# BadgerTechnologies/navigation

Measured on NVIDIA B200. Metric: ms per updateMap+inflation @4k^2 grid; DWA trajectories scored/sec, lower is better.
Workload: dtype u8

## Files before the change

### navigation_b200/csrc/dwa.cu

```cuda
#include <algorithm>
#include <cmath>
#include <cstdlib>
#include <limits>
#include <memory>
#include <vector>

#include "dwa_kernels.cuh"
#include "fleet_costmap.cuh"
#include "tp_kernels.cuh"

using namespace navgpu;

namespace {

struct P2 {
  double x, y;
};

void adjust_plan_resolution(const std::vector<P2>& in, std::vector<P2>& out, double resolution) {
  out.clear();
  if (in.empty()) return;
  double last_x = in[0].x, last_y = in[0].y;
  out.push_back(in[0]);
  const double min_sq_resolution = resolution * resolution * 4;
// ... 88 lines not shown
    NAVGPU_CUDA(cudaEventCreateWithFlags(ev, cudaEventDisableTiming));
  } else {
    NAVGPU_CUDA(cudaEventSynchronize(*ev));
  }
  memcpy(*stage, host_grid, bytes);
  NAVGPU_CUDA(cudaMemcpy2DAsync(dev, pitch, *stage, sx, sx, sy, cudaMemcpyHostToDevice, stream));
  NAVGPU_CUDA(cudaEventRecord(*ev, stream));
  return NAVGPU_OK;
}
}

struct navgpu_dwa {
  int device = 0;
  cudaStream_t stream = nullptr;
  navgpu_dwa_config cfg;
  unsigned sx = 0, sy = 0;
  double res = 0;
  uint8_t* d_cost_own = nullptr;
  const uint8_t* d_cost = nullptr;
  uint8_t* h_cost_stage = nullptr;
  cudaEvent_t ev_cost_stage = nullptr;
  unsigned pitch = 0;
  double ox = 0, oy = 0;
  DwaPlans plans;
  double* d_plan[3] = {nullptr, nullptr, nullptr};
  size_t plan_capacity[3] = {0, 0, 0};
  bool plan_dirty[3] = {false, false, false};
  bool align_aliased = false;
  DwaScales scales = {};
  uint32_t* d_dist[4] = {nullptr, nullptr, nullptr, nullptr};
  float* d_samples = nullptr;
  size_t samples_capacity = 0;
  float* h_samples_stage = nullptr;
  size_t samples_stage_capacity = 0;
  cudaEvent_t ev_samples_stage = nullptr;
  bool samples_on_device = false;
  double* d_block_cost = nullptr;
  long long* d_block_index = nullptr;
  size_t block_capacity = 0;
  unsigned int* d_counters = nullptr;
  double* d_best_cost = nullptr;
  long long* d_best_index = nullptr;
  DwaDeviceResult* h_result = nullptr;
  double* h_points = nullptr;
  double* h_best = nullptr;
  double* d_terms = nullptr;
// ... 80 lines not shown
    auto launch = [&](auto kernel) -> int {
      if (sliced_smem > 48 * 1024)
        NAVGPU_CUDA(cudaFuncSetAttribute(kernel, cudaFuncAttributeMaxDynamicSharedMemorySize, (int)sliced_smem));
      kernel<<<n_ctas, kMapGridThreads, sliced_smem, stream>>>(ma, jobs_per_robot, planes);
      return NAVGPU_OK;
    };
    switch (wpt) {
      case 1: NAVGPU_TRY(launch(k_mapgrid_prepare_sliced<1>)); break;
      case 2: NAVGPU_TRY(launch(k_mapgrid_prepare_sliced<2>)); break;
      case 3: NAVGPU_TRY(launch(k_mapgrid_prepare_sliced<3>)); break;
      default: NAVGPU_TRY(launch(k_mapgrid_prepare_sliced<4>)); break;
    }
  } else {
    const size_t mg_smem = size_t(4) * NW * sizeof(uint32_t);
    if (mg_smem > 200 * 1024) return fail(NAVGPU_ERR_UNSUPPORTED, "local costmap %ux%u too large for the MapGrid kernel", sx, sy);
    if (mg_smem > 48 * 1024)
      NAVGPU_CUDA(cudaFuncSetAttribute(k_mapgrid_prepare, cudaFuncAttributeMaxDynamicSharedMemorySize, (int)mg_smem));
    k_mapgrid_prepare<<<n_ctas, kMapGridThreads, mg_smem, stream>>>(ma, jobs_per_robot);
  }
  NAVGPU_LAUNCHED(1);
  return NAVGPU_OK;
}

int prepare_grids(navgpu_dwa* h, const DwaGeom& g) {
  for (int k = 0; k < 3; ++k) NAVGPU_TRY(upload_plan(h, k));
  MapGridArgs ma;
  ma.g = g;
  ma.allow_unknown = h->cfg.allow_unknown;
  const std::vector<P2>* adjusted = h->plans.adjusted;
  ma.job[0] = MapGridJob{h->d_plan[0], (int)adjusted[0].size(), 0, h->d_dist[0]};
  ma.job[1] = MapGridJob{h->d_plan[0], (int)adjusted[0].size(), 1, h->d_dist[1]};
  ma.job[2] = MapGridJob{h->d_plan[1], (int)adjusted[1].size(), 1, h->d_dist[2]};
  ma.job[3] = MapGridJob{h->d_plan[2], (int)adjusted[2].size(), 0, h->d_dist[3]};
  if (h->plans.align_is_path) {
    ma.job[3].dist = h->d_dist[0];
    ma.job[3].skip = 1;
  }
  ma.fleet = nullptr;
  NAVGPU_TRY(launch_mapgrid(h->sx, h->sy, h->stream, ma, 4, 4));
  h->align_aliased = h->plans.align_is_path;
  return NAVGPU_OK;
}

int critic_args(navgpu_dwa* h, const DwaGeom& g, const double* footprint_xy, int n_footprint, DwaScoreArgs& a) {
  if (n_footprint < 0 || n_footprint > kMaxFootprint) return fail(NAVGPU_ERR_UNSUPPORTED, "footprint with more than %d vertices", kMaxFootprint);
  dwa_config_args(h->cfg, h->scales, footprint_xy, n_footprint, a);
  a.scale_alignment = h->plans.alignment_scale;
  a.g = g;
  for (int k = 0; k < 4; ++k) a.dist[k] = h->d_dist[k];
  if (h->align_aliased) a.dist[3] = h->d_dist[0];
  a.osc_mask = h->osc.mask();
  return NAVGPU_OK;
}

int begin_cycle(navgpu_dwa* h, const double pose[3], const double velv[3], const double* footprint_xy, int n_footprint,
                Cycle& cy, bool prepare = true) {
  NAVGPU_TRY(use_device(h));
  if (!h->d_cost) return fail(NAVGPU_ERR_INVALID, "no costmap set");
  if (h->plans.plan.empty()) return fail(NAVGPU_ERR_INVALID, "no plan set");
  if (n_footprint < 0 || n_footprint > kMaxFootprint) return fail(NAVGPU_ERR_UNSUPPORTED, "footprint with more than %d vertices", kMaxFootprint);
  const float pos[3] = {(float)pose[0], (float)pose[1], (float)pose[2]};
  const float vel[3] = {(float)velv[0], (float)velv[1], (float)velv[2]};
  const float goal[2] = {(float)h->plans.plan.back().x, (float)h->plans.plan.back().y};
// ... 9 lines not shown
    }
    if (!h->samples_on_device || s.v != h->last_samples) {
      const size_t bytes = s.v.size() * sizeof(float);
      if (bytes > h->samples_stage_capacity) {
        if (h->h_samples_stage) cudaFreeHost(h->h_samples_stage);
        h->h_samples_stage = nullptr;
        NAVGPU_CUDA(cudaMallocHost(&h->h_samples_stage, 2 * bytes));
        h->samples_stage_capacity = 2 * bytes;
      }
      if (!h->ev_samples_stage) NAVGPU_CUDA(cudaEventCreateWithFlags(&h->ev_samples_stage, cudaEventDisableTiming));
      else NAVGPU_CUDA(cudaEventSynchronize(h->ev_samples_stage));
      memcpy(h->h_samples_stage, s.v.data(), bytes);
      NAVGPU_CUDA(cudaMemcpyAsync(h->d_samples, h->h_samples_stage, bytes, cudaMemcpyHostToDevice, h->stream));
      NAVGPU_CUDA(cudaEventRecord(h->ev_samples_stage, h->stream));
      h->samples_on_device = true;
    }
  } else {
    h->samples_on_device = false;
  }
  h->last_samples = s.v;
  h->last_nx = s.nx; h->last_ny = s.ny; h->last_nth = s.nth;

  DwaGeom g{h->d_cost, h->sx, h->sy, h->pitch, h->res, h->ox, h->oy, 1.0 / h->res};
  if (prepare) NAVGPU_TRY(prepare_grids(h, g));

  DwaScoreArgs& a = cy.args;
  NAVGPU_TRY(critic_args(h, g, footprint_xy, n_footprint, a));
  a.vxs = h->d_samples;
  a.vys = h->d_samples + s.nx;
  a.vths = h->d_samples + s.nx + s.ny;
  a.nx = s.nx; a.ny = s.ny; a.nth = s.nth;
  a.inline_samples = inline_samples ? 1 : 0;
  if (inline_samples) memcpy(a.samples_inline, s.v.data(), s.v.size() * sizeof(float));
  cy.n_samples = (long long)s.nx * s.ny * s.nth;
  a.begin = 0;
  a.end = cy.n_samples;
  a.stride_rank = 0;
  a.stride_world = 1;
  for (int k = 0; k < kShardMaxWorld; ++k) a.shard_peer[k] = nullptr;
  a.shard_seq = 0;
  for (int k = 0; k < 3; ++k) { a.pos[k] = pos[k]; a.vel[k] = vel[k]; }
  a.all_terms = nullptr;
  a.counters = h->d_counters;
  a.best_cost = h->d_best_cost;
  a.best_index = h->d_best_index;
  a.finish_out = nullptr;
  a.finish_points = nullptr;
  a.finish_capacity = 0;
  h->n_samples_last = cy.n_samples;
  return NAVGPU_OK;
// ... 56 lines not shown
  h->device = device;
  h->cfg = *cfg;
  h->sx = size_x; h->sy = size_y; h->res = resolution;
  NAVGPU_CUDA(cudaSetDevice(device));
  NAVGPU_CUDA(cudaStreamCreateWithFlags(&h->stream, cudaStreamNonBlocking));
  for (int k = 0; k < 4; ++k) NAVGPU_CUDA(cudaMalloc(&h->d_dist[k], size_t(size_x) * size_y * sizeof(uint32_t)));
  NAVGPU_CUDA(cudaMalloc(&h->d_counters, 2 * sizeof(unsigned int)));
  NAVGPU_CUDA(cudaMemset(h->d_counters, 0, 2 * sizeof(unsigned int)));
  NAVGPU_CUDA(cudaMalloc(&h->d_best_cost, sizeof(double)));
  NAVGPU_CUDA(cudaMalloc(&h->d_best_index, sizeof(long long)));
  NAVGPU_CUDA(cudaHostAlloc(&h->h_result, sizeof(DwaDeviceResult), cudaHostAllocMapped));
  NAVGPU_CUDA(cudaHostAlloc(&h->h_points, size_t(kPointsCapacity) * 3 * sizeof(double), cudaHostAllocMapped));
  NAVGPU_CUDA(cudaMallocHost(&h->h_best, 2 * sizeof(double)));
  apply_config(h.get());
  *out = h.release();
  return NAVGPU_OK;
}

int navgpu_dwa_destroy(navgpu_dwa* h) {
  if (!h) return NAVGPU_OK;
  cudaSetDevice(h->device);
  cudaStreamSynchronize(h->stream);
  cudaFree(h->d_cost_own);
  if (h->h_cost_stage) cudaFreeHost(h->h_cost_stage);
  if (h->h_samples_stage) cudaFreeHost(h->h_samples_stage);
  if (h->ev_samples_stage) cudaEventDestroy(h->ev_samples_stage);
  if (h->ev_cost_stage) cudaEventDestroy(h->ev_cost_stage);
  for (int k = 0; k < 3; ++k) cudaFree(h->d_plan[k]);
  for (int k = 0; k < 4; ++k) cudaFree(h->d_dist[k]);
  cudaFree(h->d_samples); cudaFree(h->d_block_cost); cudaFree(h->d_block_index); cudaFree(h->d_counters);
  cudaFree(h->d_best_cost); cudaFree(h->d_best_index);
  cudaFree(h->d_terms); cudaFree(h->d_reported);
  for (int r = 0; r < kShardMaxWorld; ++r)
    if (h->shard_ipc[r] && h->shard_peer[r]) cudaIpcCloseMemHandle(h->shard_peer[r]);
  cudaFree(h->d_shard);
  cudaFree(h->d_traj);
  cudaFreeHost(h->h_result); cudaFreeHost(h->h_points); cudaFreeHost(h->h_best);
  cudaStreamDestroy(h->stream);
  delete h;
  return NAVGPU_OK;
}

int navgpu_dwa_reconfigure(navgpu_dwa* h, const navgpu_dwa_config* cfg) {
  if (!h || !cfg) return fail(NAVGPU_ERR_INVALID, "bad arguments");
  h->cfg = *cfg;
  apply_config(h);
  return NAVGPU_OK;
}

int navgpu_dwa_set_costmap(navgpu_dwa* h, const uint8_t* host_grid, double origin_x, double origin_y) {
  if (!h || !host_grid) return fail(NAVGPU_ERR_INVALID, "bad arguments");
  NAVGPU_TRY(use_device(h));
  const unsigned pitch = grid_pitch(h->sx);
  if (!h->d_cost_own) NAVGPU_CUDA(cudaMalloc(&h->d_cost_own, size_t(pitch) * h->sy));
  NAVGPU_TRY(stage_grid_upload(&h->h_cost_stage, &h->ev_cost_stage, h->d_cost_own, pitch, host_grid, h->sx, h->sy, h->stream));
  h->d_cost = h->d_cost_own;
  h->pitch = pitch;
  h->ox = origin_x;
  h->oy = origin_y;
  return NAVGPU_OK;
}

int navgpu_dwa_set_costmap_device(navgpu_dwa* h, const uint8_t* dev_grid, uint32_t pitch, double origin_x, double origin_y) {
  if (!h || !dev_grid || pitch < h->sx) return fail(NAVGPU_ERR_INVALID, "bad arguments");
  h->d_cost = dev_grid;
  h->pitch = pitch;
  h->ox = origin_x;
  h->oy = origin_y;
  return NAVGPU_OK;
}

int navgpu_dwa_set_plan(navgpu_dwa* h, const double pose[3], const double* plan_xy, int n) {
  if (!h || !pose || !plan_xy || n <= 0) return fail(NAVGPU_ERR_INVALID, "bad plan");
  if (update_plan_and_local_costs(h->plans, h->cfg, h->res, pose, plan_xy, n)) h->plan_dirty[2] = true;
  h->plan_dirty[0] = h->plan_dirty[1] = true;
  return NAVGPU_OK;
}

int navgpu_dwa_reset_oscillation(navgpu_dwa* h) {
  if (!h) return fail(NAVGPU_ERR_INVALID, "null handle");
  h->osc.reset();
  return NAVGPU_OK;
// ... 109 lines not shown
    if (offsets[t + 1] < offsets[t]) return fail(NAVGPU_ERR_INVALID, "trajectory offsets must not decrease");
  const size_t b_points = size_t(n_points) * 3 * sizeof(double), b_vels = size_t(n_traj) * 3 * sizeof(double),
               b_costs = size_t(n_traj) * sizeof(double), b_terms = terms_out ? size_t(n_traj) * 6 * sizeof(double) : 0,
               b_off = size_t(n_traj + 1) * sizeof(int32_t);
  const size_t need = b_points + b_vels + b_costs + b_terms + b_off;
  if (need > h->traj_capacity) {
    if (h->d_traj) cudaFree(h->d_traj);
    h->d_traj = nullptr;
    NAVGPU_CUDA(cudaMalloc(&h->d_traj, 2 * need));
    h->traj_capacity = 2 * need;
  }
  double* d_points = reinterpret_cast<double*>(h->d_traj);
  double* d_vels = reinterpret_cast<double*>(h->d_traj + b_points);
  double* d_costs = reinterpret_cast<double*>(h->d_traj + b_points + b_vels);
  double* d_terms = terms_out ? reinterpret_cast<double*>(h->d_traj + b_points + b_vels + b_costs) : nullptr;
  int* d_off = reinterpret_cast<int*>(h->d_traj + b_points + b_vels + b_costs + b_terms);
  if (b_points) NAVGPU_CUDA(cudaMemcpyAsync(d_points, points_xyth, b_points, cudaMemcpyHostToDevice, h->stream));
  NAVGPU_CUDA(cudaMemcpyAsync(d_vels, vels, b_vels, cudaMemcpyHostToDevice, h->stream));
  NAVGPU_CUDA(cudaMemcpyAsync(d_off, offsets, b_off, cudaMemcpyHostToDevice, h->stream));
  DwaScoreArgs a;
  memset(&a, 0, sizeof(a));
  const DwaGeom g{h->d_cost, h->sx, h->sy, h->pitch, h->res, h->ox, h->oy, 1.0 / h->res};
  NAVGPU_TRY(critic_args(h, g, footprint_xy, n_footprint, a));
  const int blocks = (n_traj + kDwaWarpsPerBlock - 1) / kDwaWarpsPerBlock;
  k_dwa_score_points<<<blocks, kDwaWarpsPerBlock * 32, 0, h->stream>>>(a, d_off, d_points, d_vels, n_traj, d_costs, d_terms);
  NAVGPU_LAUNCHED(1);
  NAVGPU_CUDA(cudaGetLastError());
  NAVGPU_CUDA(cudaMemcpyAsync(costs_out, d_costs, b_costs, cudaMemcpyDeviceToHost, h->stream));
  if (terms_out) NAVGPU_CUDA(cudaMemcpyAsync(terms_out, d_terms, b_terms, cudaMemcpyDeviceToHost, h->stream));
  NAVGPU_CUDA(cudaStreamSynchronize(h->stream));
  return NAVGPU_OK;
}

int navgpu_dwa_update_oscillation(navgpu_dwa* h, const double pose[3], double cost, double xv, double yv, double thetav) {
  if (!h || !pose) return fail(NAVGPU_ERR_INVALID, "bad arguments");
  const float pos[3] = {(float)pose[0], (float)pose[1], (float)pose[2]};
  h->osc.update(pos, cost, xv, yv, thetav, h->cfg.min_trans_vel, h->cfg.oscillation_reset_dist, h->cfg.oscillation_reset_angle);
  return NAVGPU_OK;
}

int navgpu_dwa_get_samples(navgpu_dwa* h, int32_t counts_out[3], float* samples_out, int capacity) {
  if (!h || !counts_out || capacity < 0 || (capacity > 0 && !samples_out)) return fail(NAVGPU_ERR_INVALID, "bad arguments");
  counts_out[0] = h->last_nx; counts_out[1] = h->last_ny; counts_out[2] = h->last_nth;
  const size_t n = std::min<size_t>(h->last_samples.size(), (size_t)capacity);
  if (n) memcpy(samples_out, h->last_samples.data(), n * sizeof(float));
  return h->last_samples.size() > (size_t)capacity ? fail(NAVGPU_ERR_CAPACITY, "samples_out too small") : NAVGPU_OK;
// ... 259 lines not shown
  double* d_block_cost = nullptr;
  long long* d_block_index = nullptr;
  size_t blocks_capacity = 0;
  unsigned* d_generated = nullptr;
  DwaDeviceResult* d_results = nullptr;
  DwaDeviceResult* h_results = nullptr;
  bool plans_dirty = true;
  std::vector<FleetRobot> h_robots;
  std::vector<size_t> plan_off;
  bool started = false;
  FleetTp* tp = nullptr;
  std::vector<uint8_t> active;
  FleetDwaState* h_state = nullptr;
  FleetDwaState* d_state = nullptr;
  bool state_on_device = false;
  float* d_slot_samples = nullptr;
  uint8_t* d_flags = nullptr;
  char* h_records_stage = nullptr;
  cudaEvent_t ev_records_stage = nullptr;
  bool records_dirty = true;
  std::vector<FleetRobot> h_check;
  char* d_check = nullptr;
  size_t check_capacity = 0;
};

static void init_planner_scalars(navgpu_fleet* f, int n_robots, const navgpu_dwa_config* cfg, uint32_t size_x,
                                 uint32_t size_y, double resolution, const double* footprint_xy, int n_footprint,
                                 int device) {
  f->device = device;
  f->n = n_robots;
  f->sx = size_x; f->sy = size_y;
  f->res = resolution;
  f->cfg = *cfg;
  f->footprint.assign(footprint_xy, footprint_xy + 2 * n_footprint);
  f->scales = dwa_scales(*cfg, resolution);
}

static int alloc_planner_side(navgpu_fleet* f) {
  const int n_robots = f->n;
  NAVGPU_CUDA(cudaSetDevice(f->device));
  NAVGPU_CUDA(cudaMalloc(&f->d_robots, sizeof(FleetRobot) * n_robots));
  NAVGPU_CUDA(cudaMalloc(&f->d_dist, size_t(n_robots) * 4 * f->sx * f->sy * sizeof(uint32_t)));
  NAVGPU_CUDA(cudaMalloc(&f->d_generated, sizeof(unsigned) * n_robots));
  NAVGPU_CUDA(cudaMemset(f->d_generated, 0, sizeof(unsigned) * n_robots));
  NAVGPU_CUDA(cudaMalloc(&f->d_results, sizeof(DwaDeviceResult) * n_robots));
  NAVGPU_CUDA(cudaMallocHost(&f->h_results, sizeof(DwaDeviceResult) * n_robots));
// ... 47 lines not shown
  NAVGPU_CUDA(cudaStreamSynchronize(stream));
  return NAVGPU_OK;
}

template <class SetJobs>
static int fleet_upload_grids(navgpu_fleet* f, SetJobs set_jobs) {
  if (!f->grids_dirty) return NAVGPU_OK;
  for (int r = 0; r < f->n; ++r) {
    MapGridRobot& G = f->h_robots[r].grids;
    G.g = DwaGeom{f->d_master + size_t(r) * f->stride * f->pitch, f->sx, f->sy, f->pitch, f->res, f->origins[2 * r],
                  f->origins[2 * r + 1], 1.0 / f->res};
    set_jobs(r, G.job);
  }
  NAVGPU_CUDA(cudaMemcpyAsync(f->d_robots, f->h_robots.data(), sizeof(FleetRobot) * f->n, cudaMemcpyHostToDevice, f->stream));
  NAVGPU_CUDA(cudaStreamSynchronize(f->stream));
  f->grids_dirty = false;
  return NAVGPU_OK;
}

static void fleet_dwa_base_args(const navgpu_fleet* f, DwaScoreArgs& base) {
  memset(&base, 0, sizeof(base));
  base.g = DwaGeom{nullptr, f->sx, f->sy, f->pitch, f->res, 0.0, 0.0, 1.0 / f->res};
  dwa_config_args(f->cfg, f->scales, f->footprint.data(), (int)(f->footprint.size() / 2), base);
}

static int fleet_launch_mapgrid(navgpu_fleet* f, int allow_unknown, int jobs_per_robot) {
  MapGridArgs ma;
  memset(&ma, 0, sizeof(ma));
  ma.g = DwaGeom{nullptr, f->sx, f->sy, f->pitch, f->res, 0.0, 0.0, 1.0 / f->res};
  ma.allow_unknown = allow_unknown;
  ma.fleet = f->d_robots;
  return launch_mapgrid(f->sx, f->sy, f->stream, ma, jobs_per_robot * f->n, jobs_per_robot);
}

static int fleet_state_to_host(navgpu_fleet* f) {
  if (!f->state_on_device) return NAVGPU_OK;
  NAVGPU_CUDA(cudaSetDevice(f->device));
  NAVGPU_CUDA(cudaMemcpyAsync(f->h_state, f->d_state, sizeof(FleetDwaState) * f->n, cudaMemcpyDeviceToHost, f->stream));
  NAVGPU_CUDA(cudaStreamSynchronize(f->stream));
  f->state_on_device = false;
  if (f->sensing) {
    for (int r = 0; r < f->n; ++r) {
      f->origins[2 * r] = f->h_state[r].origin[0];
      f->origins[2 * r + 1] = f->h_state[r].origin[1];
    }
    fleet_costmap_set_origins(f->sensing, f->origins.data());
// ... 85 lines not shown

int navgpu_fleet_create_sensing(navgpu_fleet** out, int n_robots, const navgpu_dwa_config* cfg, uint32_t size_x,
                                uint32_t size_y, double resolution, const navgpu_fleet_costmap_config* cm,
                                const double* footprint_xy, int n_footprint, int device) {
  return create_sensing(out, n_robots, cfg, size_x, size_y, resolution, cm, nullptr, footprint_xy, n_footprint, device);
}

int navgpu_fleet_create_sensing_voxel(navgpu_fleet** out, int n_robots, const navgpu_dwa_config* cfg, uint32_t size_x,
                                      uint32_t size_y, double resolution, const navgpu_fleet_costmap_config* cm,
                                      const navgpu_fleet_voxel_config* voxel, const double* footprint_xy,
                                      int n_footprint, int device) {
  if (!voxel) return fail(NAVGPU_ERR_INVALID, "null voxel config");
  return create_sensing(out, n_robots, cfg, size_x, size_y, resolution, cm, voxel, footprint_xy, n_footprint, device);
}


int navgpu_fleet_destroy(navgpu_fleet* f) {
  if (!f) return NAVGPU_OK;
  cudaSetDevice(f->device);
  if (f->stream) cudaStreamSynchronize(f->stream);
  cudaFree(f->d_stage); cudaFree(f->d_raw); cudaFree(f->d_robots); cudaFree(f->d_plans); cudaFree(f->d_samples); cudaFree(f->d_dist);
  cudaFree(f->d_block_cost); cudaFree(f->d_block_index); cudaFree(f->d_generated); cudaFree(f->d_results);
  cudaFree(f->d_check);
  cudaFreeHost(f->h_results);
  cudaFree(f->d_state); cudaFree(f->d_slot_samples); cudaFree(f->d_flags);
  if (f->h_state) cudaFreeHost(f->h_state);
  if (f->h_records_stage) cudaFreeHost(f->h_records_stage);
  if (f->ev_records_stage) cudaEventDestroy(f->ev_records_stage);
  fleet_tp_free(f->tp);
  navgpu_costmap_destroy(f->costmap);
  fleet_costmap_destroy(f->sensing);
  delete f;
  return NAVGPU_OK;
}

int navgpu_fleet_set_maps(navgpu_fleet* f, const uint8_t* raw_maps, const double* origins_xy) {
  if (!f || !raw_maps || !origins_xy) return fail(NAVGPU_ERR_INVALID, "bad arguments");
  if (f->sensing) return fail(NAVGPU_ERR_INVALID, "a sensing fleet builds its maps from scans (navgpu_fleet_set_scans)");
  NAVGPU_CUDA(cudaSetDevice(f->device));
  f->origins.assign(origins_xy, origins_xy + size_t(2) * f->n);
  f->grids_dirty = true;
  f->records_dirty = true;
  const size_t raw_bytes = size_t(f->n) * f->sy * f->sx;
  NAVGPU_CUDA(cudaMemcpyAsync(f->d_raw, raw_maps, raw_bytes, cudaMemcpyHostToDevice, f->stream));
  {
    dim3 block(32, 8);
// ... 28 lines not shown
}

int navgpu_fleet_reset_oscillation(navgpu_fleet* f) {
  if (!f) return fail(NAVGPU_ERR_INVALID, "null handle");
  if (f->tp) return fail(NAVGPU_ERR_INVALID, "a TrajectoryPlanner fleet has no DWA oscillation flags (see navgpu_fleet_step_tp's flags)");
  NAVGPU_TRY(fleet_state_to_host(f));
  for (int r = 0; r < f->n; ++r) f->h_state[r].osc.reset();
  return NAVGPU_OK;
}

int navgpu_fleet_step(navgpu_fleet* f, const double* poses, const double* vels, navgpu_dwa_result* results) {
  if (!f || !poses || !vels || !results) return fail(NAVGPU_ERR_INVALID, "bad arguments");
  if (f->tp) return fail(NAVGPU_ERR_INVALID, "a TrajectoryPlanner fleet steps with navgpu_fleet_step_tp");
  f->started = true;
  NAVGPU_TRY(fleet_state_to_host(f));
  NAVGPU_CUDA(cudaSetDevice(f->device));
  const navgpu_dwa_config& c = f->cfg;
  const int n = f->n;
  NAVGPU_TRY(fleet_costmap_front(f, poses));
  NAVGPU_TRY(fleet_dwa_upload_plans(f));

  NAVGPU_TRY(fleet_upload_grids(f, [f](int r, MapGridJob* job) { fleet_dwa_jobs(f, r, job); }));
  if (f->sensing) NAVGPU_TRY(fleet_costmap_enqueue(f->sensing));
  NAVGPU_TRY(fleet_launch_mapgrid(f, c.allow_unknown, 4));

  std::vector<float>& samples = f->h_samples;
  samples.clear();
  int max_samples = 0;
  for (int r = 0; r < n; ++r) {
    FleetRobot& R = f->h_robots[r];
    if (!f->active[r]) {
      R.nx = R.ny = R.nth = 0;
      R.samples_offset = (int)samples.size();
      continue;
    }
    const float pos[3] = {(float)poses[3 * r], (float)poses[3 * r + 1], (float)poses[3 * r + 2]};
    const float vel[3] = {(float)vels[3 * r], (float)vels[3 * r + 1], (float)vels[3 * r + 2]};
    const float goal[2] = {(float)f->plans[r].plan.back().x, (float)f->plans[r].plan.back().y};
    const Samples s = enumerate_samples(c, pos, vel, goal);
    if (s.v.size() > (size_t)kInlineSamples) {
      cudaStreamSynchronize(f->stream);
      return fail(NAVGPU_ERR_UNSUPPORTED, "more than %d per-axis samples per robot", kInlineSamples);
    }
    for (int k = 0; k < 3; ++k) { R.pos[k] = pos[k]; R.vel[k] = vel[k]; }
    R.osc_mask = f->h_state[r].osc.mask();
    R.scale_alignment = f->plans[r].alignment_scale;
// ... 109 lines not shown
                          f->origins[2 * r + 1], 1.0 / f->res};
      fleet_dwa_jobs(f, r, R.grids.job);
      R.scale_alignment = f->plans[r].alignment_scale;
      stage[r] = R;
      flags[r] = (f->active[r] ? kFleetActive : 0) | (f->plans[r].align_is_path ? kFleetAligned : 0);
    }
    NAVGPU_CUDA(cudaMemcpyAsync(f->d_robots, stage, sizeof(FleetRobot) * n, cudaMemcpyHostToDevice, f->stream));
    NAVGPU_CUDA(cudaMemcpyAsync(f->d_flags, flags, n, cudaMemcpyHostToDevice, f->stream));
    NAVGPU_CUDA(cudaEventRecord(f->ev_records_stage, f->stream));
    f->records_dirty = f->grids_dirty = false;
  }

  const unsigned robot_ctas = (unsigned)((n + kFleetRobotThreads - 1) / kFleetRobotThreads);
  FleetPrepareArgs pa;
  pa.poses = poses; pa.vels = vels;
  pa.robots = f->d_robots; pa.state = f->d_state; pa.flags = f->d_flags;
  pa.samples = f->d_slot_samples; pa.slot = (int)slot; pa.n = n;
  pa.cfg = c;
  pa.steps = f->sensing ? fleet_costmap_device_steps(f->sensing) : nullptr;
  pa.sx = f->sx; pa.sy = f->sy; pa.res = f->res;
  k_fleet_prepare<<<robot_ctas, kFleetRobotThreads, 0, f->stream>>>(pa);
  NAVGPU_LAUNCHED(1);
  if (f->sensing) NAVGPU_TRY(fleet_costmap_enqueue(f->sensing, true));
  NAVGPU_TRY(fleet_launch_mapgrid(f, c.allow_unknown, 4));
  DwaScoreArgs base;
  fleet_dwa_base_args(f, base);
  k_fleet_score<<<(unsigned)blocks, kDwaWarpsPerBlock * 32, 0, f->stream>>>(base, f->d_robots, f->d_slot_samples, (int)bpr,
                                                                          f->d_block_cost, f->d_block_index, f->d_generated);
  k_fleet_finish<<<n, 32, 0, f->stream>>>(base, f->d_robots, f->d_slot_samples, (int)bpr, f->d_block_cost,
                                          f->d_block_index, f->d_generated, f->d_results);
  k_fleet_apply<<<robot_ctas, kFleetRobotThreads, 0, f->stream>>>(c, poses, f->d_robots, f->d_flags, f->d_results,
                                                                  f->d_state, results, n);
  NAVGPU_LAUNCHED(3);
  NAVGPU_CUDA(cudaGetLastError());
  return NAVGPU_OK;
}

int navgpu_fleet_get_costmap(navgpu_fleet* f, int robot, uint8_t* host_out) {
  if (!f || robot < 0 || robot >= f->n || !host_out) return fail(NAVGPU_ERR_INVALID, "bad arguments");
  if (f->sensing) return fleet_costmap_get(f->sensing, robot, true, host_out);
  return navgpu_costmap_get_window(f->costmap, 0, (int)(robot * f->stride), (int)f->sx, (int)(robot * f->stride + f->sy), host_out);
}

int navgpu_fleet_get_oscillation_mask(navgpu_fleet* f, int robot, int* mask_out) {
  if (!f || robot < 0 || robot >= f->n || !mask_out) return fail(NAVGPU_ERR_INVALID, "bad arguments");
  if (f->tp) return fail(NAVGPU_ERR_INVALID, "a TrajectoryPlanner fleet has no DWA oscillation flags (see navgpu_fleet_step_tp's flags)");
// ... 133 lines not shown
```

### navigation_b200/csrc/dwa_kernels.cuh

```cuda
#pragma once

#include <cstddef>

#include "common.cuh"
#include "fleet_costmap.cuh"

namespace navgpu {

constexpr int kMaxFootprint = 16;
constexpr int kInlineSamples = 640;
constexpr int kDwaWarpsPerBlock = 8;

struct DwaGeom {
  const uint8_t* cost;
  unsigned sx, sy, pitch;
  double res, ox, oy;
  double inv_res;
};

__device__ __forceinline__ int exact_cell(double d, double res, double inv_res) {
  const double q = d * inv_res;
  const double r = rint(q);
  if (fabs(q - r) <= 1e-6) {
    const int ri = (int)r;
// ... 745 lines not shown
};

struct DwaScoreArgs {
  DwaGeom g;
  const uint32_t* dist[4];
  const float* vxs;
  const float* vys;
  const float* vths;
  int nx, ny, nth;
  int inline_samples;
  float samples_inline[kInlineSamples];
  long long begin, end;
  int stride_rank, stride_world;
  ShardExchange* shard_peer[kShardMaxWorld];
  unsigned long long shard_seq;
  float pos[3], vel[3], acc[3];
  double min_trans_vel, max_trans_vel, min_rot_vel;
  double sim_time, sim_granularity, angular_sim_granularity;
  int use_dwa, sum_scores, allow_unknown, osc_mask;
  double scale_obstacle, scale_goal_front, scale_alignment, scale_path, scale_goal;
  double xshift;
  int nfp;
  double fpx[kMaxFootprint], fpy[kMaxFootprint];
  double* all_terms;
  double* block_cost;
  long long* block_index;
  unsigned int* counters;
  double* best_cost;
  long long* best_index;
  DwaDeviceResult* finish_out;
  double* finish_points;
  int finish_capacity;
};

struct TrajResult {
  double cost;
  bool generated;
  int num_steps;
};

__device__ __forceinline__ double nan_quiet() { return __longlong_as_double(0x7ff8000000000000ll); }

template <class Args>
__device__ __forceinline__ int footprint_vertex_cell(const Args& a, double x, double y, double cos_th, double sin_th,
                                                     int v) {
  const double wx = x + (a.fpx[v] * cos_th - a.fpy[v] * sin_th), wy = y + (a.fpx[v] * sin_th + a.fpy[v] * cos_th);
// ... 26 lines not shown
        off += minor;
      }
      off += major;
    }
  } else {
    for (int k = 0; k <= den; ++k) {
      best = max(best, (int)cost[off]);
      num += numadd;
      if (num >= den) {
        num -= den;
        off += minor;
      }
      off += major;
    }
  }
  const bool bad = a.allow_unknown ? lethal_probe == 0 : best >= kLethal;
  return bad ? -1 : best;
}
template <class Args>
__device__ __forceinline__ int footprint_edge_cost(const Args& a, int cell_p, int cell_q) {
  return footprint_edge_cost(a, a.g.cost, cell_p, cell_q);
}

struct CriticAcc {
  bool obst_fail;
  double obst_sum, obst_last;
  double grid_code[4], grid_last[4];
};
__device__ __forceinline__ void critic_acc_init(CriticAcc& acc) {
  acc.obst_fail = false;
  acc.obst_sum = acc.obst_last = 0.0;
#pragma unroll
  for (int k = 0; k < 4; ++k) acc.grid_code[k] = acc.grid_last[k] = 0.0;
}

__device__ __forceinline__ void score_round(const DwaScoreArgs& a, const uint8_t* __restrict__ cost, int lane, int cnt,
                                            double px, double py, double c, double s, double* warp_scratch,
                                            CriticAcc& acc) {
  const bool active = lane < cnt;
  double* pose_s = warp_scratch;
  unsigned* edge_max = reinterpret_cast<unsigned*>(warp_scratch + 128);
  pose_s[lane] = px;
  pose_s[32 + lane] = py;
  pose_s[64 + lane] = c;
  pose_s[96 + lane] = s;
  edge_max[lane] = 0;
  __syncwarp();
  double occ = 0.0;
  bool fail = false;
  if (a.nfp >= 3) {
    int* vcell = reinterpret_cast<int*>(warp_scratch + 128 + 16);
    const int items = cnt * a.nfp;
    const unsigned inv_nfp = (65536u + (unsigned)a.nfp - 1u) / (unsigned)a.nfp;
    for (int it = lane; it < items; it += 32) {
      const int p = (int)(((unsigned)it * inv_nfp) >> 16), v = it - p * a.nfp;
      vcell[it] = footprint_vertex_cell(a, pose_s[p], pose_s[32 + p], pose_s[64 + p], pose_s[96 + p], v);
    }
    __syncwarp();
    for (int it = lane; it < items; it += 32) {
      const int p = (int)(((unsigned)it * inv_nfp) >> 16), e = it - p * a.nfp;
      const int next = e + 1 < a.nfp ? it + 1 : it - e;
      const int ec = footprint_edge_cost(a, cost, vcell[it], vcell[next]);
      atomicMax(&edge_max[p], ec < 0 ? 0x80000000u : (unsigned)ec);
    }
    __syncwarp();
  }
  int cell0_x = 0, cell0_y = 0, cell1_x = 0, cell1_y = 0;
  bool on_map0 = false, on_map1 = false;
  if (active) {
    on_map0 = dwa_world_to_map(a.g, px, py, cell0_x, cell0_y);
    if (a.xshift != 0.0) {
      on_map1 = dwa_world_to_map(a.g, px + a.xshift * c, py + a.xshift * s, cell1_x, cell1_y);
    } else {
      on_map1 = on_map0; cell1_x = cell0_x; cell1_y = cell0_y;
    }
  }
  if (active) {
    const int cx = cell0_x, cy = cell0_y;
    if (a.nfp == 0 || !on_map0) fail = true;
    else {
      const int centre = cost[cy * (int)a.g.pitch + cx];
      int f = (int)edge_max[lane];
      if (a.nfp < 3) {
        f = (centre == kLethal || centre == kInscribed || (centre == kNoInfo && !a.allow_unknown)) ? -1 : centre;
      }
      if (f < 0) fail = true;
      else occ = fmax(fmax(0.0, (double)f), (double)centre);
    }
  }
  acc.obst_fail |= __any_sync(0xffffffffu, fail);
  double ssum = occ;
#pragma unroll
  for (int o = 16; o > 0; o >>= 1) ssum += __shfl_xor_sync(0xffffffffu, ssum, o);
  acc.obst_sum += ssum;
  acc.obst_last = __shfl_sync(0xffffffffu, occ, cnt - 1);
  __syncwarp();
  cudaGridDependencySynchronize();
#pragma unroll
  for (int k = 0; k < 4; ++k) {
    const bool shifted = k >= 2;
    const bool stop_on_failure = k < 2;
    double code = 0.0, d = 0.0;
    if (active) {
      const int cx = shifted ? cell1_x : cell0_x, cy = shifted ? cell1_y : cell0_y;
      if (!(shifted ? on_map1 : on_map0)) code = -4.0;
// ... 137 lines not shown
    float x = sx, y = sy, my_x = sx, my_y = sy;
    warp_scratch[lane] = ddx;
    warp_scratch[32 + lane] = ddy;
    __syncwarp();
    for (int l = 0; l < cnt; ++l) {
      if (lane == l) { my_x = x; my_y = y; }
      const double dxl = warp_scratch[l], dyl = warp_scratch[32 + l];
      x = (float)((double)x + dxl);
      y = (float)((double)y + dyl);
    }
    __syncwarp();
    sx = x;
    sy = y;
    sth = th;

    const bool active = lane < cnt;
    const double px = my_x, py = my_y;
    if (points_out && active && base + lane < points_capacity) {
      points_out[3 * (base + lane)] = px;
      points_out[3 * (base + lane) + 1] = py;
      points_out[3 * (base + lane) + 2] = thd;
    }
    if (!kScore) continue;
    score_round(a, cost, lane, cnt, px, py, c, s, warp_scratch, acc);
  }

  if (!kScore) return res;
  res.cost = combine_critics(a, osc_bad, acc, terms_out, lane);
  return res;
}

__device__ void finish_winner(const DwaScoreArgs& a, long long idx, double cost, DwaDeviceResult* out, double* points,
                              int points_capacity, double* warp_scratch, unsigned* n_generated) {
  const int lane = threadIdx.x & 31;
  TrajResult r;
  r.generated = false;
  r.num_steps = 0;
  if (idx >= 0) r = score_sample<false>(a, idx, lane, nullptr, points, points_capacity, warp_scratch, a.g.cost);
  if (lane == 0) {
    out->n_scored = (int)*n_generated;
    *n_generated = 0;
    if (idx >= 0 && r.generated && cost >= 0) {
      const int ith = (int)(idx % a.nth);
      const long long t1 = idx / a.nth;
      const int iy = (int)(t1 % a.ny), ix = (int)(t1 / a.ny);
      float vx = sample_vx(a, ix), vy = sample_vy(a, iy), vth = sample_vth(a, ith);
      if (!a.use_dwa) {
// ... 185 lines not shown

__global__ void __launch_bounds__(kDwaWarpsPerBlock * 32) k_dwa_score_points(DwaScoreArgs a, const int* __restrict__ offsets,
                                                                           const double* __restrict__ points,
                                                                           const double* __restrict__ vels, int n_traj,
                                                                           double* __restrict__ costs_out,
                                                                           double* __restrict__ terms_out) {
  __shared__ double s_scratch[kDwaWarpsPerBlock][kWarpScratchDoubles];
  const int lane = threadIdx.x & 31, warp = threadIdx.x >> 5;
  const int t = blockIdx.x * kDwaWarpsPerBlock + warp;
  if (t >= n_traj) return;
  const int first = offsets[t], n = offsets[t + 1] - first;
  const bool osc_bad = oscillation_rejects(a.osc_mask, vels[3 * t], vels[3 * t + 1], vels[3 * t + 2]);
  CriticAcc acc;
  critic_acc_init(acc);
  for (int base = 0; base < n; base += 32) {
    const int cnt = min(32, n - base);
    double px = 0.0, py = 0.0, c = 1.0, s = 0.0;
    if (lane < cnt) {
      const double* p = points + 3 * (size_t)(first + base + lane);
      px = p[0];
      py = p[1];
      sincos(p[2], &s, &c);
    }
    score_round(a, a.g.cost, lane, cnt, px, py, c, s, s_scratch[warp], acc);
    __syncwarp();
  }
  const double total = combine_critics(a, osc_bad, acc, terms_out ? terms_out + 6 * (size_t)t : nullptr, lane);
  if (lane == 0) costs_out[t] = total;
}

__global__ void k_dwa_finish(DwaScoreArgs a, long long forced_index, double forced_cost, DwaDeviceResult* out,
                             double* points, int points_capacity) {
  __shared__ double s_scratch[kWarpScratchDoubles];
  finish_winner(a, forced_index, forced_cost, out, points, points_capacity, s_scratch, &a.counters[1]);
}

__global__ void k_dwa_report(const double* __restrict__ terms, double* __restrict__ reported, long long n) {
  __shared__ double s_full[1024];
  __shared__ double s_prefix[1024];
  __shared__ double s_carry;
  if (threadIdx.x == 0) s_carry = -1.0;
  __syncthreads();
  for (long long base = 0; base < n; base += blockDim.x) {
    const long long i = base + threadIdx.x;
    double t[6];
    double full = nan_quiet();
    bool gen = false;
// ... 18 lines not shown
        if (f != INFINITY && (best < 0 || f < best)) best = f;
      }
      s_carry = best;
    }
    __syncthreads();
    if (i < n) {
      double rep = nan_quiet();
      if (gen) {
        const double best = s_prefix[threadIdx.x];
        rep = 0.0;
        for (int k = 0; k < 6; ++k) {
          if (t[k] < 0) { rep = t[k]; break; }
          rep += t[k];
          if (best > 0 && rep > best) break;
        }
      }
      reported[i] = rep;
    }
    __syncthreads();
  }
}


__device__ __forceinline__ void fleet_patch_args(DwaScoreArgs& s_a, const DwaScoreArgs& base, const FleetRobot& r,
                                                 const float* samples) {
  const uint32_t* src = reinterpret_cast<const uint32_t*>(&base);
  uint32_t* dst = reinterpret_cast<uint32_t*>(&s_a);
  constexpr int kHeadWords = (int)(offsetof(DwaScoreArgs, samples_inline) / 4);
  constexpr int kTailStart = (int)((offsetof(DwaScoreArgs, samples_inline) + sizeof(float) * kInlineSamples) / 4);
  constexpr int kWords = (int)(sizeof(DwaScoreArgs) / 4);
  for (int i = threadIdx.x; i < kHeadWords; i += blockDim.x) dst[i] = src[i];
  for (int i = kTailStart + threadIdx.x; i < kWords; i += blockDim.x) dst[i] = src[i];
  const int n_s = r.nx + r.ny + r.nth;
  for (int i = threadIdx.x; i < n_s; i += blockDim.x) s_a.samples_inline[i] = samples[r.samples_offset + i];
  __syncthreads();
  if (threadIdx.x == 0) {
    s_a.g = r.grids.g;
    for (int k = 0; k < 4; ++k) s_a.dist[k] = r.grids.job[k].dist;
    s_a.nx = r.nx; s_a.ny = r.ny; s_a.nth = r.nth;
    s_a.inline_samples = 1;
    for (int k = 0; k < 3; ++k) { s_a.pos[k] = r.pos[k]; s_a.vel[k] = r.vel[k]; }
    s_a.osc_mask = r.osc_mask;
    s_a.scale_alignment = r.scale_alignment;
    s_a.begin = 0;
    s_a.end = (long long)r.nx * r.ny * r.nth;
    s_a.all_terms = nullptr;
    s_a.finish_out = nullptr;
  }
  __syncthreads();
}

__global__ void __launch_bounds__(kDwaWarpsPerBlock * 32, 4) k_fleet_score(DwaScoreArgs base, const FleetRobot* robots,
                                                                        const float* samples, int blocks_per_robot,
                                                                        double* block_cost, long long* block_index,
                                                                        unsigned* generated) {
  __shared__ DwaScoreArgs s_a;
  __shared__ double s_cost[kDwaWarpsPerBlock];
  __shared__ long long s_index[kDwaWarpsPerBlock];
  __shared__ int s_generated[kDwaWarpsPerBlock];
  __shared__ double s_scratch[kDwaWarpsPerBlock][kWarpScratchDoubles];
  const int robot = blockIdx.x / blocks_per_robot, local = blockIdx.x % blocks_per_robot;
  const FleetRobot& r = robots[robot];
  if ((long long)local * kDwaWarpsPerBlock >= (long long)r.nx * r.ny * r.nth) {
    if (threadIdx.x == 0) {
      block_cost[blockIdx.x] = INFINITY;
      block_index[blockIdx.x] = -1;
    }
    return;
  }
  fleet_patch_args(s_a, base, r, samples);
  const uint8_t* costmap = s_a.g.cost;
  const int lane = threadIdx.x & 31, warp = threadIdx.x >> 5;
  const long long sample = (long long)local * kDwaWarpsPerBlock + warp;
  double cost = INFINITY;
  long long index = -1;
  int gen = 0;
  if (sample < s_a.end) {
    const TrajResult t = score_sample<true>(s_a, sample, lane, nullptr, nullptr, 0, s_scratch[warp], costmap);
    gen = t.generated;
    if (t.generated && t.cost >= 0) {
      cost = t.cost;
      index = sample;
    }
  }
  if (lane == 0) {
    s_cost[warp] = cost;
    s_index[warp] = index;
    s_generated[warp] = gen;
  }
  __syncthreads();
  if (threadIdx.x == 0) {
    double bc = INFINITY;
    long long bi = -1;
// ... 13 lines not shown

__global__ void k_fleet_scatter_maps(const uint8_t* __restrict__ raw, uint8_t* __restrict__ stacked, unsigned sx,
                                     unsigned sy, unsigned stride, unsigned pitch, unsigned n) {
  const size_t row = (size_t)blockIdx.x * blockDim.y + threadIdx.y;
  if (row >= (size_t)n * sy) return;
  const unsigned r = (unsigned)(row / sy), y = (unsigned)(row - (size_t)r * sy);
  const uint8_t* src = raw + row * sx;
  uint8_t* dst = stacked + ((size_t)r * stride + y) * pitch;
  if ((sx & 3u) == 0 && (((size_t)src) & 3u) == 0) {
    for (unsigned x = threadIdx.x * 4; x < sx; x += blockDim.x * 4)
      *reinterpret_cast<uint32_t*>(dst + x) = *reinterpret_cast<const uint32_t*>(src + x);
  } else {
    for (unsigned x = threadIdx.x; x < sx; x += blockDim.x) dst[x] = src[x];
  }
}

__global__ void __launch_bounds__(32) k_fleet_finish(DwaScoreArgs base, const FleetRobot* robots, const float* samples,
                                                     int blocks_per_robot, const double* block_cost,
                                                     const long long* block_index, unsigned* generated,
                                                     DwaDeviceResult* results) {
  __shared__ DwaScoreArgs s_a;
  __shared__ double s_scratch[kWarpScratchDoubles];
  const int robot = blockIdx.x, lane = threadIdx.x;
  fleet_patch_args(s_a, base, robots[robot], samples);
  double bc = INFINITY;
  long long bi = -1;
  for (int i = lane; i < blocks_per_robot; i += 32) {
    const double c = block_cost[(size_t)robot * blocks_per_robot + i];
    const long long ix = block_index[(size_t)robot * blocks_per_robot + i];
    if (ix >= 0 && (bi < 0 || better(c, ix, bc, bi))) {
      bc = c;
      bi = ix;
    }
  }
#pragma unroll
  for (int o = 16; o > 0; o >>= 1) {
    const double oc = __shfl_xor_sync(0xffffffffu, bc, o);
    const long long oi = __shfl_xor_sync(0xffffffffu, bi, o);
    if (oi >= 0 && (bi < 0 || better(oc, oi, bc, bi))) {
      bc = oc;
      bi = oi;
    }
  }
  finish_winner(s_a, bi, bc, results + robot, nullptr, 0, s_scratch, generated + robot);
}

__global__ void __launch_bounds__(32, 1) k_fleet_check(DwaScoreArgs base, const FleetRobot* robots,
                                                    const int* __restrict__ robot_of, const float* __restrict__ candidates,
                                                    double* __restrict__ costs) {
  __shared__ DwaScoreArgs s_a;
  __shared__ double s_scratch[kWarpScratchDoubles];
  const int c = blockIdx.x;
  fleet_patch_args(s_a, base, robots[robot_of[c]], candidates + 3 * (size_t)c);
  const TrajResult r = score_sample<true>(s_a, 0, threadIdx.x & 31, nullptr, nullptr, 0, s_scratch, s_a.g.cost);
  if (threadIdx.x == 0) costs[c] = r.generated ? r.cost : ((s_a.nfp == 0 && s_a.scale_obstacle != 0.0) ? -9.0 : 0.0);
}

constexpr int kFleetRobotThreads = 128;
constexpr uint8_t kFleetActive = 1, kFleetAligned = 2;

struct FleetPrepareArgs {
  const double* poses;
  const double* vels;
  FleetRobot* robots;
  FleetDwaState* state;
  const uint8_t* flags;
  float* samples;
  int slot, n;
  navgpu_dwa_config cfg;
  FleetCmStep* steps;
  unsigned sx, sy;
  double res;
};

__global__ void __launch_bounds__(kFleetRobotThreads) k_fleet_prepare(FleetPrepareArgs a) {
  const int r = blockIdx.x * blockDim.x + threadIdx.x;
// ... 46 lines not shown
```

Baseline: 0.03790.

## Skip footprint edge walks using precomputed obstacle-free clearance bitmap

Adds a kernel that builds a per-map bit-packed clearance mask by dilating lethal/unknown cells by the footprint's circumscribed reach, using separable shift-OR passes in shared memory. During trajectory scoring, poses whose centre cell is clear skip the per-vertex footprint edge rasterization. Only the remaining poses are compacted into the warp scratch, and the last pose of a trajectory is always walked. This aims to cut the dominant footprint-cost work at the price of an extra dilation kernel per costmap change and an extra bitmap lookup per pose.

New measurement: 0.03811 (median of 6 runs). No clear change (+0.6%).

```diff
diff --git a/navigation_b200/csrc/dwa.cu b/navigation_b200/csrc/dwa.cu
--- a/navigation_b200/csrc/dwa.cu
+++ b/navigation_b200/csrc/dwa.cu
@@ -134,6 +134,8 @@
   cudaEvent_t ev_cost_stage = nullptr;
   unsigned pitch = 0;
   double ox = 0, oy = 0;
+  uint32_t* d_clear = nullptr;
+  int clear_reach = 0, clear_allow_unknown = 0;
   DwaPlans plans;
   double* d_plan[3] = {nullptr, nullptr, nullptr};
   size_t plan_capacity[3] = {0, 0, 0};
@@ -260,6 +262,30 @@
   return NAVGPU_OK;
 }
 
+int footprint_clear_reach(const navgpu_dwa_config& c, double res, const double* footprint_xy, int n_footprint) {
+  if (c.sum_scores || n_footprint < 3) return 0;
+  double rmax = 0.0;
+  for (int k = 0; k < n_footprint; ++k) {
+    const double r = std::hypot(footprint_xy[2 * k], footprint_xy[2 * k + 1]);
+    if (!(r <= kClearMaxReach * res)) return 0;
+    rmax = std::max(rmax, r);
+  }
+  const double reach = std::ceil(rmax / res) + 1.0;
+  return reach <= kClearMaxReach ? (int)reach : 0;
+}
+
+int launch_footprint_clear(const uint8_t* grid, size_t grid_stride, unsigned pitch, unsigned sx, unsigned sy, int reach,
+                           int allow_unknown, uint32_t* clear, int n_maps, cudaStream_t stream, bool* built) {
+  const size_t smem = size_t(2) * clear_words(sx) * sy * sizeof(uint32_t);
+  *built = smem <= (size_t)kClearMaxSmem;
+  if (!*built) return NAVGPU_OK;
+  if (smem > 48 * 1024)
+    NAVGPU_CUDA(cudaFuncSetAttribute(k_footprint_clear, cudaFuncAttributeMaxDynamicSharedMemorySize, (int)smem));
+  k_footprint_clear<<<n_maps, kClearThreads, smem, stream>>>(grid, grid_stride, pitch, sx, sy, reach, allow_unknown, clear);
+  NAVGPU_LAUNCHED(1);
+  return NAVGPU_OK;
+}
+
 int prepare_grids(navgpu_dwa* h, const DwaGeom& g) {
   for (int k = 0; k < 3; ++k) NAVGPU_TRY(upload_plan(h, k));
   MapGridArgs ma;
@@ -277,6 +303,24 @@
   ma.fleet = nullptr;
   NAVGPU_TRY(launch_mapgrid(h->sx, h->sy, h->stream, ma, 4, 4));
   h->align_aliased = h->plans.align_is_path;
+  return NAVGPU_OK;
+}
+
+int footprint_clear(navgpu_dwa* h, const double* footprint_xy, int n_footprint, const uint32_t** clear) {
+  *clear = nullptr;
+  const int reach = footprint_clear_reach(h->cfg, h->res, footprint_xy, n_footprint);
+  if (reach == 0) return NAVGPU_OK;
+  if (h->d_cost != h->d_cost_own || reach != h->clear_reach || h->cfg.allow_unknown != h->clear_allow_unknown) {
+    h->clear_reach = 0;
+    if (!h->d_clear) NAVGPU_CUDA(cudaMalloc(&h->d_clear, size_t(clear_words(h->sx)) * h->sy * sizeof(uint32_t)));
+    bool built;
+    NAVGPU_TRY(launch_footprint_clear(h->d_cost, 0, h->pitch, h->sx, h->sy, reach, h->cfg.allow_unknown, h->d_clear, 1,
+                                      h->stream, &built));
+    if (!built) return NAVGPU_OK;
+    h->clear_reach = reach;
+    h->clear_allow_unknown = h->cfg.allow_unknown;
+  }
+  *clear = h->d_clear;
   return NAVGPU_OK;
 }
 
@@ -332,10 +376,13 @@
   h->last_nx = s.nx; h->last_ny = s.ny; h->last_nth = s.nth;
 
   DwaGeom g{h->d_cost, h->sx, h->sy, h->pitch, h->res, h->ox, h->oy, 1.0 / h->res};
+  const uint32_t* clear;
+  NAVGPU_TRY(footprint_clear(h, footprint_xy, n_footprint, &clear));
   if (prepare) NAVGPU_TRY(prepare_grids(h, g));
 
   DwaScoreArgs& a = cy.args;
   NAVGPU_TRY(critic_args(h, g, footprint_xy, n_footprint, a));
+  a.clear = clear;
   a.vxs = h->d_samples;
   a.vys = h->d_samples + s.nx;
   a.vths = h->d_samples + s.nx + s.ny;
@@ -438,6 +485,7 @@
   cudaSetDevice(h->device);
   cudaStreamSynchronize(h->stream);
   cudaFree(h->d_cost_own);
+  cudaFree(h->d_clear);
   if (h->h_cost_stage) cudaFreeHost(h->h_cost_stage);
   if (h->h_samples_stage) cudaFreeHost(h->h_samples_stage);
   if (h->ev_samples_stage) cudaEventDestroy(h->ev_samples_stage);
@@ -474,6 +522,7 @@
   h->pitch = pitch;
   h->ox = origin_x;
   h->oy = origin_y;
+  h->clear_reach = 0;
   return NAVGPU_OK;
 }
 
@@ -629,6 +678,7 @@
   memset(&a, 0, sizeof(a));
   const DwaGeom g{h->d_cost, h->sx, h->sy, h->pitch, h->res, h->ox, h->oy, 1.0 / h->res};
   NAVGPU_TRY(critic_args(h, g, footprint_xy, n_footprint, a));
+  NAVGPU_TRY(footprint_clear(h, footprint_xy, n_footprint, &a.clear));
   const int blocks = (n_traj + kDwaWarpsPerBlock - 1) / kDwaWarpsPerBlock;
   k_dwa_score_points<<<blocks, kDwaWarpsPerBlock * 32, 0, h->stream>>>(a, d_off, d_points, d_vels, n_traj, d_costs, d_terms);
   NAVGPU_LAUNCHED(1);
@@ -934,6 +984,8 @@
   std::vector<FleetRobot> h_check;
   char* d_check = nullptr;
   size_t check_capacity = 0;
+  uint32_t* d_clear = nullptr;
+  bool clear_built = false;
 };
 
 static void init_planner_scalars(navgpu_fleet* f, int n_robots, const navgpu_dwa_config* cfg, uint32_t size_x,
@@ -1027,6 +1079,17 @@
   memset(&base, 0, sizeof(base));
   base.g = DwaGeom{nullptr, f->sx, f->sy, f->pitch, f->res, 0.0, 0.0, 1.0 / f->res};
   dwa_config_args(f->cfg, f->scales, f->footprint.data(), (int)(f->footprint.size() / 2), base);
+  base.clear = f->clear_built ? f->d_clear : nullptr;
+}
+
+static int fleet_footprint_clear(navgpu_fleet* f) {
+  const int reach = footprint_clear_reach(f->cfg, f->res, f->footprint.data(), (int)(f->footprint.size() / 2));
+  f->clear_built = false;
+  if (reach == 0) return NAVGPU_OK;
+  if (!f->d_clear)
+    NAVGPU_CUDA(cudaMalloc(&f->d_clear, size_t(f->n) * clear_words(f->sx) * f->sy * sizeof(uint32_t)));
+  return launch_footprint_clear(f->d_master, size_t(f->stride) * f->pitch, f->pitch, f->sx, f->sy, reach,
+                                f->cfg.allow_unknown, f->d_clear, f->n, f->stream, &f->clear_built);
 }
 
 static int fleet_launch_mapgrid(navgpu_fleet* f, int allow_unknown, int jobs_per_robot) {
@@ -1158,6 +1221,7 @@
   cudaFree(f->d_stage); cudaFree(f->d_raw); cudaFree(f->d_robots); cudaFree(f->d_plans); cudaFree(f->d_samples); cudaFree(f->d_dist);
   cudaFree(f->d_block_cost); cudaFree(f->d_block_index); cudaFree(f->d_generated); cudaFree(f->d_results);
   cudaFree(f->d_check);
+  cudaFree(f->d_clear);
   cudaFreeHost(f->h_results);
   cudaFree(f->d_state); cudaFree(f->d_slot_samples); cudaFree(f->d_flags);
   if (f->h_state) cudaFreeHost(f->h_state);
@@ -1232,6 +1296,7 @@
 
   NAVGPU_TRY(fleet_upload_grids(f, [f](int r, MapGridJob* job) { fleet_dwa_jobs(f, r, job); }));
   if (f->sensing) NAVGPU_TRY(fleet_costmap_enqueue(f->sensing));
+  NAVGPU_TRY(fleet_footprint_clear(f));
   NAVGPU_TRY(fleet_launch_mapgrid(f, c.allow_unknown, 4));
 
   std::vector<float>& samples = f->h_samples;
@@ -1387,6 +1452,7 @@
   k_fleet_prepare<<<robot_ctas, kFleetRobotThreads, 0, f->stream>>>(pa);
   NAVGPU_LAUNCHED(1);
   if (f->sensing) NAVGPU_TRY(fleet_costmap_enqueue(f->sensing, true));
+  NAVGPU_TRY(fleet_footprint_clear(f));
   NAVGPU_TRY(fleet_launch_mapgrid(f, c.allow_unknown, 4));
   DwaScoreArgs base;
   fleet_dwa_base_args(f, base);
diff --git a/navigation_b200/csrc/dwa_kernels.cuh b/navigation_b200/csrc/dwa_kernels.cuh
--- a/navigation_b200/csrc/dwa_kernels.cuh
+++ b/navigation_b200/csrc/dwa_kernels.cuh
@@ -791,6 +791,7 @@
   double xshift;
   int nfp;
   double fpx[kMaxFootprint], fpy[kMaxFootprint];
+  const uint32_t* clear;
   double* all_terms;
   double* block_cost;
   long long* block_index;
@@ -863,6 +864,62 @@
   return footprint_edge_cost(a, a.g.cost, cell_p, cell_q);
 }
 
+constexpr int kClearMaxReach = 63;
+constexpr int kClearThreads = 256;
+constexpr int kClearMaxSmem = 160 * 1024;
+
+__host__ __device__ inline int clear_words(unsigned sx) { return (int)((sx + 31) / 32); }
+__device__ __forceinline__ int clear_step(int covered, int reach) { return min(covered + 1, reach - covered); }
+
+__global__ void __launch_bounds__(kClearThreads) k_footprint_clear(const uint8_t* __restrict__ grid, size_t grid_stride,
+                                                                   unsigned pitch, unsigned sx, unsigned sy, int reach,
+                                                                   int allow_unknown, uint32_t* __restrict__ clear) {
+  extern __shared__ uint32_t s_planes[];
+  const int W = clear_words(sx), NW = W * (int)sy;
+  uint32_t* A = s_planes;
+  uint32_t* B = s_planes + NW;
+  const uint8_t* cost = grid + blockIdx.x * grid_stride;
+  const int lane = threadIdx.x & 31;
+  for (int i = threadIdx.x >> 5; i < NW; i += kClearThreads / 32) {
+    const int y = i / W, x = (i - y * W) * 32 + lane;
+    bool bad = true;
+    if (x < (int)sx) {
+      const int c = cost[(size_t)y * pitch + x];
+      bad = c == kLethal || (c == kNoInfo && !allow_unknown);
+    }
+    const unsigned word = __ballot_sync(0xffffffffu, bad);
+    if (lane == 0) A[i] = word;
+  }
+  __syncthreads();
+  for (int c = 0, r; c < reach; c += r) {
+    r = clear_step(c, reach);
+    for (int i = threadIdx.x; i < NW; i += kClearThreads) {
+      const int w = i % W;
+      const uint32_t mid = A[i], lo = w > 0 ? A[i - 1] : ~0u, hi = w + 1 < W ? A[i + 1] : ~0u;
+      B[i] = mid | __funnelshift_rc(mid, hi, r) | __funnelshift_lc(lo, mid, r);
+    }
+    __syncthreads();
+    uint32_t* t = A; A = B; B = t;
+  }
+  for (int c = 0, r; c < reach; c += r) {
+    r = clear_step(c, reach);
+    for (int i = threadIdx.x; i < NW; i += kClearThreads) {
+      const int y = i / W;
+      B[i] = A[i] | (y >= r ? A[i - r * W] : ~0u) | (y + r < (int)sy ? A[i + r * W] : ~0u);
+    }
+    __syncthreads();
+    uint32_t* t = A; A = B; B = t;
+  }
+  uint32_t* out = clear + (size_t)blockIdx.x * NW;
+  for (int i = threadIdx.x; i < NW; i += kClearThreads) out[i] = ~A[i];
+}
+
+__device__ __forceinline__ unsigned lanemask_lt() {
+  unsigned m;
+  asm("mov.u32 %0, %%lanemask_lt;" : "=r"(m));
+  return m;
+}
+
 struct CriticAcc {
   bool obst_fail;
   double obst_sum, obst_last;
@@ -876,22 +933,31 @@
 }
 
 __device__ __forceinline__ void score_round(const DwaScoreArgs& a, const uint8_t* __restrict__ cost, int lane, int cnt,
-                                            double px, double py, double c, double s, double* warp_scratch,
-                                            CriticAcc& acc) {
+                                            bool last_round, double px, double py, double c, double s,
+                                            double* warp_scratch, CriticAcc& acc) {
   const bool active = lane < cnt;
+  bool walk = active && a.nfp >= 3;
+  int cx, cy;
+  if (walk && a.clear && !(last_round && lane == cnt - 1) && dwa_world_to_map(a.g, px, py, cx, cy))
+    walk = !((a.clear[cy * clear_words(a.g.sx) + (cx >> 5)] >> (cx & 31)) & 1u);
+  const unsigned walkers = __ballot_sync(0xffffffffu, walk);
   double* pose_s = warp_scratch;
   unsigned* edge_max = reinterpret_cast<unsigned*>(warp_scratch + 128);
-  pose_s[lane] = px;
-  pose_s[32 + lane] = py;
-  pose_s[64 + lane] = c;
-  pose_s[96 + lane] = s;
-  edge_max[lane] = 0;
-  __syncwarp();
   double occ = 0.0;
   bool fail = false;
-  if (a.nfp >= 3) {
+  unsigned f_edges = 0;
+  if (walkers) {
+    if (walk) {
+      const int slot = __popc(walkers & lanemask_lt());
+      pose_s[slot] = px;
+      pose_s[32 + slot] = py;
+      pose_s[64 + slot] = c;
+      pose_s[96 + slot] = s;
+      edge_max[slot] = 0;
+    }
+    __syncwarp();
     int* vcell = reinterpret_cast<int*>(warp_scratch + 128 + 16);
-    const int items = cnt * a.nfp;
+    const int items = __popc(walkers) * a.nfp;
     const unsigned inv_nfp = (65536u + (unsigned)a.nfp - 1u) / (unsigned)a.nfp;
     for (int it = lane; it < items; it += 32) {
       const int p = (int)(((unsigned)it * inv_nfp) >> 16), v = it - p * a.nfp;
@@ -905,6 +971,7 @@
       atomicMax(&edge_max[p], ec < 0 ? 0x80000000u : (unsigned)ec);
     }
     __syncwarp();
+    if ((walkers >> lane) & 1u) f_edges = edge_max[__popc(walkers & lanemask_lt())];
   }
   int cell0_x = 0, cell0_y = 0, cell1_x = 0, cell1_y = 0;
   bool on_map0 = false, on_map1 = false;
@@ -921,7 +988,7 @@
     if (a.nfp == 0 || !on_map0) fail = true;
     else {
       const int centre = cost[cy * (int)a.g.pitch + cx];
-      int f = (int)edge_max[lane];
+      int f = (int)f_edges;
       if (a.nfp < 3) {
         f = (centre == kLethal || centre == kInscribed || (centre == kNoInfo && !a.allow_unknown)) ? -1 : centre;
       }
@@ -1105,7 +1172,7 @@
       points_out[3 * (base + lane) + 2] = thd;
     }
     if (!kScore) continue;
-    score_round(a, cost, lane, cnt, px, py, c, s, warp_scratch, acc);
+    score_round(a, cost, lane, cnt, base + 32 >= num_steps, px, py, c, s, warp_scratch, acc);
   }
 
   if (!kScore) return res;
@@ -1337,7 +1404,7 @@
       py = p[1];
       sincos(p[2], &s, &c);
     }
-    score_round(a, a.g.cost, lane, cnt, px, py, c, s, s_scratch[warp], acc);
+    score_round(a, a.g.cost, lane, cnt, base + 32 >= n, px, py, c, s, s_scratch[warp], acc);
     __syncwarp();
   }
   const double total = combine_critics(a, osc_bad, acc, terms_out ? terms_out + 6 * (size_t)t : nullptr, lane);
@@ -1402,8 +1469,8 @@
 }
 
 
-__device__ __forceinline__ void fleet_patch_args(DwaScoreArgs& s_a, const DwaScoreArgs& base, const FleetRobot& r,
-                                                 const float* samples) {
+__device__ __forceinline__ void fleet_patch_args(DwaScoreArgs& s_a, const DwaScoreArgs& base, int robot,
+                                                 const FleetRobot& r, const float* samples) {
   const uint32_t* src = reinterpret_cast<const uint32_t*>(&base);
   uint32_t* dst = reinterpret_cast<uint32_t*>(&s_a);
   constexpr int kHeadWords = (int)(offsetof(DwaScoreArgs, samples_inline) / 4);
@@ -1426,6 +1493,7 @@
     s_a.end = (long long)r.nx * r.ny * r.nth;
     s_a.all_terms = nullptr;
     s_a.finish_out = nullptr;
+    if (base.clear) s_a.clear = base.clear + (size_t)robot * clear_words(base.g.sx) * base.g.sy;
   }
   __syncthreads();
 }
@@ -1448,7 +1516,7 @@
     }
     return;
   }
-  fleet_patch_args(s_a, base, r, samples);
+  fleet_patch_args(s_a, base, robot, r, samples);
   const uint8_t* costmap = s_a.g.cost;
   const int lane = threadIdx.x & 31, warp = threadIdx.x >> 5;
   const long long sample = (long long)local * kDwaWarpsPerBlock + warp;
@@ -1508,7 +1576,7 @@
   __shared__ DwaScoreArgs s_a;
   __shared__ double s_scratch[kWarpScratchDoubles];
   const int robot = blockIdx.x, lane = threadIdx.x;
-  fleet_patch_args(s_a, base, robots[robot], samples);
+  fleet_patch_args(s_a, base, robot, robots[robot], samples);
   double bc = INFINITY;
   long long bi = -1;
   for (int i = lane; i < blocks_per_robot; i += 32) {
@@ -1536,8 +1604,8 @@
                                                     double* __restrict__ costs) {
   __shared__ DwaScoreArgs s_a;
   __shared__ double s_scratch[kWarpScratchDoubles];
-  const int c = blockIdx.x;
-  fleet_patch_args(s_a, base, robots[robot_of[c]], candidates + 3 * (size_t)c);
+  const int c = blockIdx.x, robot = robot_of[c];
+  fleet_patch_args(s_a, base, robot, robots[robot], candidates + 3 * (size_t)c);
   const TrajResult r = score_sample<true>(s_a, 0, threadIdx.x & 31, nullptr, nullptr, 0, s_scratch, s_a.g.cost);
   if (threadIdx.x == 0) costs[c] = r.generated ? r.cost : ((s_a.nfp == 0 && s_a.scale_obstacle != 0.0) ? -9.0 : 0.0);
 }
```
